# BichenWuUCB/squeezeDet

Hardware: NVIDIA H100
Metric: images/sec (1242x375, b=20) (higher is better)
Workload: dtype f32 (3xTF32 wgmma, fp32 accumulate)

## Files before the change

include/sqdet_b200.h:

```cpp
#ifndef SQDET_B200_H_
#define SQDET_B200_H_

#include <stdint.h>

#ifdef __cplusplus
extern "C" {
#endif

#define SQDET_OK                 0
#define SQDET_ERR_INVALID_ARG   (-1)
#define SQDET_ERR_CUDA          (-2)
#define SQDET_ERR_UNSUPPORTED   (-3)
#define SQDET_ERR_STATE         (-4)
#define SQDET_ERR_NOT_FOUND     (-5)
#define SQDET_ERR_OVERFLOW      (-6)

#define SQDET_PAD_SAME   0
#define SQDET_PAD_VALID  1

#define SQDET_MATH_FP32_SIMT   0
#define SQDET_MATH_TF32X3_TC   1

typedef struct sqdet_engine sqdet_engine;

// ... 32 lines not shown
                      int size, int stride, int relu, int conv_with_bias, int* out);
int sqdet_add_pool(sqdet_engine* e, const char* layer_name, int src, int size,
                   int stride, int padding, int* out);
int sqdet_add_fire(sqdet_engine* e, const char* layer_name, int src, int s1x1,
                   int e1x1, int e3x3, int* out);
int sqdet_add_add_relu(sqdet_engine* e, const char* name, int a, int b, int* out);
int sqdet_set_preds(sqdet_engine* e, int preds, const double* anchor_box, int64_t num_anchors);
int sqdet_finalize(sqdet_engine* e);

int sqdet_num_params(sqdet_engine* e);
int sqdet_param_info(sqdet_engine* e, int index, char* name_buf, int name_cap,
                     int64_t shape[4], int* ndim);
int sqdet_set_param(sqdet_engine* e, const char* name, const float* data,
                    const int64_t* shape, int ndim);

int sqdet_num_tensors(sqdet_engine* e);
int sqdet_tensor_info(sqdet_engine* e, int id, char* name_buf, int name_cap,
                      int64_t shape[4]);
int sqdet_read_tensor(sqdet_engine* e, int id, float* host_out);
int sqdet_num_ops(sqdet_engine* e);
int sqdet_op_info(sqdet_engine* e, int index, char* name_buf, int name_cap,
                  int64_t* flops, int64_t* params, int64_t* min_bytes);
int sqdet_op_k_split(sqdet_engine* e, int index);

int sqdet_forward(sqdet_engine* e, const float* images_dev, void* stream);
int sqdet_forward_n(sqdet_engine* e, const float* images_dev, int n, void* stream);
int sqdet_forward_u8(sqdet_engine* e, const uint8_t* images_dev, int n, void* stream);
int sqdet_forward_profiled(sqdet_engine* e, const float* images_dev, void* stream,
                           float* op_ms);
int sqdet_results_dev(sqdet_engine* e, float** det_boxes, float** det_probs,
                      int64_t** det_class, sqdet_det** dets, int32_t** counts,
                      int32_t* max_dets);
int sqdet_detect(sqdet_engine* e, const float* images, float* det_boxes,
                 float* det_probs, int64_t* det_class, sqdet_det* dets,
                 int32_t* counts, void* stream);
#define SQDET_IMG_F32 0
#define SQDET_IMG_U8  1
int sqdet_set_bgr_means(sqdet_engine* e, const double bgr_means[3]);
int sqdet_submit(sqdet_engine* e, const void* images, int img_type, sqdet_det* dets,
                 int32_t* counts);
int sqdet_wait(sqdet_engine* e);
int sqdet_submit_frames(sqdet_engine* e, const uint8_t* const* frames,
                        const int32_t* heights, const int32_t* widths, int order,
                        int rescale, sqdet_det* dets, int32_t* counts);
int sqdet_submit_frames_n(sqdet_engine* e, int n, const uint8_t* const* frames,
                          const int32_t* heights, const int32_t* widths, int order,
// ... 28 lines not shown
int sqdet_comm_unique_id(void* id128);
int sqdet_comm_init(sqdet_engine* e, int nranks, int rank, const void* id128);
int sqdet_comm_attach(sqdet_engine* e, void* nccl_comm, int nranks, int rank);
int sqdet_comm_destroy(sqdet_engine* e);
int sqdet_set_gather_in_forward(sqdet_engine* e, int on);
int sqdet_allgather(sqdet_engine* e, void* nccl_comm, void* stream);
int sqdet_gathered_dev(sqdet_engine* e, void** gathered_dev, int64_t* bytes_per_rank,
                       int32_t* nranks);

int sqdet_conv2d(const float* x_dev, const float* w_hwio_dev, const float* bias_dev,
                 const float* scale_dev, const float* shift_dev, float* y_dev,
                 int B, int H, int W, int Cin, int Cout, int size, int stride,
                 int padding, int relu, int y_cstride, int y_coff, int math_mode,
                 void* stream);
int sqdet_conv2d_k_split(const float* x_dev, const float* w_hwio_dev, const float* bias_dev,
                         const float* scale_dev, const float* shift_dev, float* y_dev,
                         int B, int H, int W, int Cin, int Cout, int size, int stride,
                         int padding, int relu, int y_cstride, int y_coff, int math_mode,
                         int k_split, void* stream);
int sqdet_fire(const float* x_dev, const float* w_sq_dev, const float* b_sq_dev,
               const float* w_e1_dev, const float* b_e1_dev, const float* w_e3_dev,
               const float* b_e3_dev, float* y_dev, int B, int H, int W, int Cin, int S,
               int E1, int E3, int math_mode, void* stream);
int sqdet_maxpool_nhwc(const float* x_dev, float* y_dev, int B, int H, int W, int C,
                       int size, int stride, int padding, void* stream);
#define SQDET_PRE_RESIZE_THEN_SUB 0
#define SQDET_PRE_SUB_THEN_RESIZE 1
int sqdet_preprocess_u8(const uint8_t* src_dev, int src_h, int src_w, float* dst_dev,
                        int dst_h, int dst_w, const double* bgr_means, int order,
                        void* stream);
int sqdet_interpret(const float* preds_dev, const float* anchors_f32_dev,
                    float* det_boxes_dev, float* det_probs_dev, int64_t* det_class_dev,
                    int B, int grid_h, int grid_w, int anchors_per_grid, int classes,
                    int image_width, int image_height, float exp_thresh, void* stream);
int sqdet_topk_nms(const float* boxes_dev, const float* probs_dev,
                   const int64_t* cls_dev, int B, int A, int classes, int top_n,
                   float prob_thresh, float nms_thresh, sqdet_det* dets_dev,
                   int32_t* counts_dev, int max_dets, void* stream);
int sqdet_merge_tiles(const float* boxes_dev, const float* probs_dev, const int64_t* cls_dev,
                      int A, int t, const int32_t* tile_frames, const int32_t* tile_xy, int n,
                      int classes, int top_n, float prob_thresh, float nms_thresh,
                      sqdet_det* dets_dev, int32_t* counts_dev, int max_dets, void* stream);
typedef struct sqdet_draw_style {
  int32_t            classes;
  const char* const* class_names;
  const uint8_t*     class_bgr;
// ... 60 lines not shown
```

squeezedet_b200/_lib.py:

```python
from __future__ import annotations

import ctypes as C
import os

import numpy as np

_HERE = os.path.dirname(os.path.abspath(__file__))
LIB_PATH = os.path.join(_HERE, 'lib', 'libsqdet_b200.so')

OK = 0
PAD_SAME, PAD_VALID = 0, 1
MATH_FP32_SIMT, MATH_TF32X3_TC = 0, 1
IMG_F32, IMG_U8 = 0, 1
_PAD = {'SAME': PAD_SAME, 'VALID': PAD_VALID}


class SqdetError(RuntimeError):
  def __init__(self, code, msg):
    super().__init__('sqdet error %d: %s' % (code, msg))
    self.code = code


class Det(C.Structure):
  _fields_ = [('anchor', C.c_int32), ('cls', C.c_int32), ('prob', C.c_float),
# ... 35 lines not shown

SIGNATURES = {
    'sqdet_last_error': (C.c_char_p, []),
    'sqdet_version': (C.c_char_p, []),
    'sqdet_device_count': (_i, []),
    'sqdet_create': (_i, [C.POINTER(Config), _i, C.POINTER(_vp)]),
    'sqdet_destroy': (_i, [_vp]),
    'sqdet_add_conv': (_i, [_vp, C.c_char_p, _i, _i, _i, _i, _i, _i, _ip]),
    'sqdet_add_conv_bn': (_i, [_vp, C.c_char_p, _i, _i, _i, _i, _i, _i, _ip]),
    'sqdet_add_pool': (_i, [_vp, C.c_char_p, _i, _i, _i, _i, _ip]),
    'sqdet_add_fire': (_i, [_vp, C.c_char_p, _i, _i, _i, _i, _ip]),
    'sqdet_add_add_relu': (_i, [_vp, C.c_char_p, _i, _i, _ip]),
    'sqdet_set_preds': (_i, [_vp, _i, _vp, _i64]),
    'sqdet_finalize': (_i, [_vp]),
    'sqdet_num_params': (_i, [_vp]),
    'sqdet_param_info': (_i, [_vp, _i, C.c_char_p, _i, _i64p, _ip]),
    'sqdet_set_param': (_i, [_vp, C.c_char_p, _fp, _i64p, _i]),
    'sqdet_num_tensors': (_i, [_vp]),
    'sqdet_tensor_info': (_i, [_vp, _i, C.c_char_p, _i, _i64p]),
    'sqdet_read_tensor': (_i, [_vp, _i, _fp]),
    'sqdet_num_ops': (_i, [_vp]),
    'sqdet_op_info': (_i, [_vp, _i, C.c_char_p, _i, _i64p, _i64p, _i64p]),
    'sqdet_op_k_split': (_i, [_vp, _i]),
    'sqdet_forward': (_i, [_vp, _fp, _vp]),
    'sqdet_forward_n': (_i, [_vp, _fp, _i, _vp]),
    'sqdet_forward_u8': (_i, [_vp, _vp, _i, _vp]),
    'sqdet_forward_profiled': (_i, [_vp, _fp, _vp, _fp]),
    'sqdet_results_dev': (_i, [_vp, C.POINTER(_vp), C.POINTER(_vp), C.POINTER(_vp),
                               C.POINTER(_vp), C.POINTER(_vp), C.POINTER(C.c_int32)]),
    'sqdet_detect': (_i, [_vp, _fp, _fp, _fp, _fp, _fp, _fp, _vp]),
    'sqdet_set_bgr_means': (_i, [_vp, _vp]),
    'sqdet_submit': (_i, [_vp, _vp, _i, _vp, _vp]),
    'sqdet_wait': (_i, [_vp]),
    'sqdet_submit_frames': (_i, [_vp, _vp, _vp, _vp, _i, _i, _vp, _vp]),
    'sqdet_submit_frames_n': (_i, [_vp, _i, _vp, _vp, _vp, _i, _i, _vp, _vp]),
    'sqdet_forward_frames_u8': (_i, [_vp, _i, _vp, _vp, _vp, _vp, _i, _i, _vp]),
    'sqdet_forward_frames_nv12': (_i, [_vp, _i, _vp, _vp, _vp, _vp, _vp, _vp, _vp, _i, _i, _vp]),
    'sqdet_forward_frames': (_i, [_vp, _i, _i, _vp, _vp, _vp, _vp, _vp, _i, _i, _vp]),
    'sqdet_forward_tiles': (_i, [_vp, _i, _i, _vp, _vp, _vp, _vp, _i, _vp, _i, _vp]),
    'sqdet_tile_results_dev': (_i, [_vp, C.POINTER(_vp), C.POINTER(_vp), C.POINTER(C.c_int32)]),
    'sqdet_set_box_scale': (_i, [_vp, _vp]),
    'sqdet_launches_per_forward': (_i, [_vp]),
    'sqdet_engine_stream': (_vp, [_vp]),
    'sqdet_comm_unique_id': (_i, [_vp]),
    'sqdet_comm_init': (_i, [_vp, _i, _i, _vp]),
    'sqdet_comm_attach': (_i, [_vp, _vp, _i, _i]),
    'sqdet_comm_destroy': (_i, [_vp]),
    'sqdet_set_gather_in_forward': (_i, [_vp, _i]),
    'sqdet_allgather': (_i, [_vp, _vp, _vp]),
    'sqdet_gathered_dev': (_i, [_vp, C.POINTER(_vp), C.POINTER(C.c_int64),
                                C.POINTER(C.c_int32)]),
    'sqdet_fire': (_i, [_fp] * 8 + [_i] * 8 + [_vp]),
    'sqdet_conv2d': (_i, [_fp, _fp, _fp, _fp, _fp, _fp] + [_i] * 12 + [_vp]),
    'sqdet_conv2d_k_split': (_i, [_fp, _fp, _fp, _fp, _fp, _fp] + [_i] * 13 + [_vp]),
    'sqdet_maxpool_nhwc': (_i, [_fp, _fp] + [_i] * 7 + [_vp]),
    'sqdet_preprocess_u8': (_i, [_vp, _i, _i, _fp, _i, _i, _vp, _i, _vp]),
    'sqdet_interpret': (_i, [_fp, _fp, _fp, _fp, _fp] + [_i] * 7 + [_f, _vp]),
    'sqdet_topk_nms': (_i, [_fp, _fp, _fp, _i, _i, _i, _i, _f, _f, _fp, _fp, _i, _vp]),
    'sqdet_merge_tiles': (_i, [_fp, _fp, _fp, _i, _i, _vp, _vp, _i, _i, _i, _f, _f, _fp, _fp, _i,
                               _vp]),
    'sqdet_draw_dets': (_i, [_i, _i, _vp, _vp, _vp, _vp, _vp, _vp, _vp, _i, C.POINTER(DrawStyle),
                             _vp]),
    'sqdet_jpeg_max_bytes': (_i64, [_i, _i]),
    'sqdet_jpeg_scratch_bytes': (_i64, [_i, _vp, _vp, _vp]),
    'sqdet_encode_jpeg': (_i, [_i, _i, _vp, _vp, _vp, _vp, _vp, _i, _vp, _i64, _vp, _vp, _i64, _vp]),
    'sqdet_jpeg_parse': (_i, [_vp, _i64, C.POINTER(JpegInfo)]),
    'sqdet_jpeg_decode_staging_bytes': (_i64, [_i, _vp, _vp]),
    'sqdet_jpeg_decode_scratch_bytes': (_i64, [_i, _vp, _vp]),
    'sqdet_decode_jpeg': (_i, [_i, _vp, _vp, _vp, _vp, _vp, _i64, _vp, _i64, _vp, _vp]),
    'sqdet_jpeg_decode_set_subsequence_bits': (_i, [_i]),
    'sqdet_malloc': (_i, [_i, _i64, C.POINTER(_vp)]),
    'sqdet_free': (_i, [_i, _vp]),
    'sqdet_malloc_host': (_i, [_i64, C.POINTER(_vp)]),
    'sqdet_free_host': (_i, [_vp]),
    'sqdet_memcpy_h2d': (_i, [_vp, _vp, _i64, _vp]),
    'sqdet_memcpy_d2h': (_i, [_vp, _vp, _i64, _vp]),
    'sqdet_stream_sync': (_i, [_i, _vp]),
# ... 141 lines not shown
```

squeezedet_b200/csrc/conv_tc.cu:

```cuda
#include <cuda.h>
#include <cuda_runtime.h>
#include <stdint.h>
#include <stdlib.h>
#include <string.h>

#include <vector>

#include "common.cuh"
#include "conv_tc.cuh"

namespace sqdet {
namespace {

constexpr int TILE_M = 128;
constexpr int NUM_THREADS = 256;
constexpr int STAGES = 3;
constexpr int MAX_CHUNKS = 32;
constexpr int FT_W = 16, FQ_W = FT_W + 2, FQ_P = 10 * FQ_W;

enum TcMode { TC_ROWS, TC_GATHER, TC_HALO, TC_FIRE };

struct TcChunk {
  int ksize, pad_t, pad_l;
  int nk;
  int ncount;
  int y_off;
  int p_off;
  long long w_off;
};

struct TcParams {
  CUtensorMap amap, amap1;
  const float* x;
  float* y;
  const float* w;
  const float* bias;
  const float* scale;
  const float* shift;
  int B, H, W, Cin, Ho, Wo, stride, relu, y_cstride;
  long long M;
  int tiles_w, tiles_h;
  int nchunks;
  TcChunk chunks[MAX_CHUNKS];
};

__device__ __forceinline__ uint32_t smem_u32(const void* p) {
  return static_cast<uint32_t>(__cvta_generic_to_shared(p));
}
__device__ __forceinline__ void cp_async4(uint32_t dst, const void* src, bool valid) {
  asm volatile("cp.async.ca.shared.global [%0], [%1], 4, %2;" ::"r"(dst), "l"(src),
// ... 275 lines not shown
  return {rest / tiles_h, rest % tiles_h * 8, tx * FT_W};
}

__device__ __forceinline__ float finish(const TcParams& p, const TcChunk& ch, int c, float v) {
  if (p.bias) v += p.bias[ch.p_off + c];
  if (p.scale) v = v * p.scale[ch.p_off + c] + p.shift[ch.p_off + c];
  if (p.relu) v = fmaxf(v, 0.f);
  return v;
}

template <typename Value>
__device__ __forceinline__ void store_pair(float* yrow, int c, int ncount, bool pair, Value value) {
  if (pair && c + 1 < ncount) {
    *reinterpret_cast<float2*>(yrow + c) = make_float2(value(c), value(c + 1));
  } else {
    if (c < ncount) yrow[c] = value(c);
    if (c + 1 < ncount) yrow[c + 1] = value(c + 1);
  }
}
__device__ __forceinline__ bool rows_pair_aligned(const TcParams& p, const TcChunk& ch) {
  return ((p.y_cstride | ch.y_off) & 1) == 0 && (reinterpret_cast<uintptr_t>(p.y) & 7) == 0;
}

template <int NT, int KC, int MODE, bool KSPLIT = false>
__global__ void __launch_bounds__(NUM_THREADS, 2)
conv_tc_kernel(const __grid_constant__ TcParams p) {
  static_assert(!KSPLIT || MODE == TC_HALO, "the K split walks halo-mode channel chunks");
  constexpr int NACC = NT / 2;
  constexpr int WST = 2 * NT * KC;
  constexpr uint32_t W_BYTES = WST * 4, TILE_BYTES = TILE_M * KC * 4, HALO_BYTES = FQ_P * KC * 4;
  constexpr int HROWS = halo_rows(KC);
  extern __shared__ __align__(16) uint8_t smem_raw[];
  float* const smem = reinterpret_cast<float*>(smem_raw + ((1024 - (smem_u32(smem_raw) & 1023)) & 1023));
  float* const sa = smem + STAGES * WST;
  uint64_t* const full = reinterpret_cast<uint64_t*>(sa + STAGES * TILE_M * KC);
  uint64_t* const empty = full + STAGES;

  const TcChunk& ch = p.chunks[blockIdx.y];
  const int tid = threadIdx.x;
  const int wg = tid >> 7, wq = (tid >> 5) & 3, lane = tid & 31, g = lane >> 2, t = lane & 3;
  const float* wch = p.w + ch.w_off;
  int k0 = 0, nk = ch.nk;
  const int taps = ch.ksize * ch.ksize;
  if (KSPLIT) {
    const int nc = ch.nk / taps, S = gridDim.z, z = blockIdx.z;
    k0 = z * nc / S * taps;
    nk = (z + 1) * nc / S * taps - k0;
    wch += (size_t)k0 * WST;
  }

// ... 64 lines not shown
  const int arow0 = wg * 64 + wq * 16 + g;
  const int r = wg * 4 + wq;
  float acc[2][NACC], sum[NACC];
#pragma unroll
  for (int i = 0; i < NACC; ++i) acc[0][i] = acc[1][i] = sum[i] = 0.f;

  for (int kk = 0; kk < nk; ++kk) {
    if (kk + STAGES - 1 < nk) load_stage(kk + STAGES - 1);
    const int s = ring_wait_full(full, kk);

    const float* tile = sa + s * TILE_M * KC;
    int prow = arow0;
    if (MODE == TC_HALO && taps > 1) {
      const int c = kk / 9, tap = kk - c * 9;
      tile = sa + (c & 1) * HROWS * KC;
      prow = (r + tap / 3) * FQ_W + g + tap % 3;
    }
    mma_chunk<NT, KC, NT != 72>(
        [&](int ks, uint32_t(&ahi)[4], uint32_t(&alo)[4]) { load_split_swz<KC>(tile, prow, ks, t, ahi, alo); },
        smem_u32(smem + s * WST), acc, sum);
    ring_release(empty, kk);
  }

  if constexpr (KSPLIT) {
    static_assert(TILE_M * NT <= STAGES * (WST + TILE_M * KC), "the partial tile fits in the ring");
    float* const part = smem;
    __syncthreads();
#pragma unroll
    for (int h = 0; h < 2; ++h)
#pragma unroll
      for (int j = 0; j < NT / 8; ++j)
        *reinterpret_cast<float2*>(part + (arow0 + 8 * h) * NT + 8 * j + 2 * t) =
            make_float2(sum[4 * j + 2 * h], sum[4 * j + 2 * h + 1]);
    cluster_sync();
    constexpr int G = TILE_M * NT / 4;
    const int S = gridDim.z, z = blockIdx.z;
    const HaloTile tl = halo_tile(p.tiles_w, p.tiles_h);
    for (int i = z * G / S + tid; i < (z + 1) * G / S; i += NUM_THREADS) {
      const uint32_t at = smem_u32(part + 4 * i);
      float4 v = ld_cluster_f4(at, 0);
      for (int q = 1; q < S; ++q) {
        const float4 u = ld_cluster_f4(at, q);
        v.x += u.x, v.y += u.y, v.z += u.z, v.w += u.w;
      }
      const int px = 4 * i / NT, c0 = 4 * i % NT;
      const int oy = tl.oy0 + px / FT_W, ox = tl.ox0 + px % FT_W;
      if (oy >= p.Ho || ox >= p.Wo) continue;
      float* yrow = p.y + (((size_t)tl.n * p.Ho + oy) * p.Wo + ox) * p.y_cstride + ch.y_off;
      const float vs[4] = {v.x, v.y, v.z, v.w};
#pragma unroll
      for (int e = 0; e < 4; ++e)
        if (c0 + e < ch.ncount) yrow[c0 + e] = finish(p, ch, c0 + e, vs[e]);
    }
    cluster_sync();
  } else {
    const bool pair = rows_pair_aligned(p, ch);
#pragma unroll
    for (int h = 0; h < 2; ++h) {
      long long m = m0 + arow0 + 8 * h;
      if (MODE == TC_HALO) {
        const HaloTile tl = halo_tile(p.tiles_w, p.tiles_h);
        const int oy = tl.oy0 + r, ox = tl.ox0 + g + 8 * h;
        if (oy >= p.Ho || ox >= p.Wo) continue;
        m = ((long long)tl.n * p.Ho + oy) * p.Wo + ox;
      } else if (m >= p.M) {
        continue;
      }
      float* yrow = p.y + (size_t)m * p.y_cstride + ch.y_off;
#pragma unroll
      for (int j = 0; j < NT / 8; ++j)
        store_pair(yrow, 8 * j + 2 * t, ch.ncount, pair,
                   [&](int c) { return finish(p, ch, c, sum[4 * j + 2 * h + (c & 1)]); });
    }
  }
}

constexpr int FS = 16;
constexpr int FQ_ROWS = 192;

__host__ __device__ constexpr int fire_stage_floats(int KCI) { return 2 * FS * KCI + FQ_ROWS * KCI; }
constexpr size_t fire_smem_bytes(int KCI) {
  return 1024 + ((size_t)STAGES * fire_stage_floats(KCI) + FQ_ROWS * (FS + 4)) * sizeof(float) +
         2 * STAGES * sizeof(uint64_t);
}

template <int KCI>
__global__ void __launch_bounds__(NUM_THREADS, 2)
fire_tc_kernel(const __grid_constant__ TcParams p) {
  constexpr int QP = FS + 4;
  constexpr int SQW = 2 * FS * KCI;
  constexpr int STAGE = fire_stage_floats(KCI);
  constexpr uint32_t SQW_BYTES = SQW * 4, HALO_BYTES = FQ_P * KCI * 4, EX_BYTES = 2 * 64 * FS * 4;
  static_assert(EX_BYTES <= (SQW + FQ_P * KCI) * 4, "expand tile fits before the zeroed rows");
  static_assert(SQW_BYTES % 1024 == 0 && STAGE * 4 % 1024 == 0, "A tiles keep the swizzle's alignment");
  extern __shared__ __align__(16) uint8_t smem_raw[];
// ... 138 lines not shown
}

TcKernel conv_tc_instance(int NT, int KC, int mode) {
  if (NT == 72) return mode == TC_HALO ? conv_tc_kernel<72, 32, TC_HALO> : conv_tc_kernel<72, 32, TC_ROWS>;
  if (mode == TC_GATHER) return conv_tc_instance<32, TC_GATHER>(NT);
  if (mode == TC_HALO)
    return KC == 32 ? conv_tc_instance<32, TC_HALO>(NT) : conv_tc_instance<16, TC_HALO>(NT);
  return KC == 32 ? conv_tc_instance<32, TC_ROWS>(NT) : conv_tc_instance<16, TC_ROWS>(NT);
}

struct PlanGroup {
  ConvGroup conv;
  int NT, KC, cin, chunk0;
};

}

struct TcImpl {
  TcParams prm{};
  int KC = 0;
  int mode = TC_ROWS;
  TcKernel kernel = nullptr;
  int ksplit = 1;
  size_t smem_bytes = 0;
  std::vector<PlanGroup> groups;
  int cout_total = 0;
  float* d_w = nullptr;
  float* d_bias = nullptr;
  float* d_scale = nullptr;
  float* d_shift = nullptr;
  long long w_floats = 0;
  const float* map_x = nullptr;
  int map_n = 0;
};

static inline float host_rn_tf32(float x) {
  uint32_t u;
  memcpy(&u, &x, 4);
  u = (u + 0x1000u) & 0xFFFFE000u;
  float r;
  memcpy(&r, &u, 4);
  return r;
}

static int pick_nt(const std::vector<ConvGroup>& groups, int KC, bool gather) {
  int best = 0;
// ... 83 lines not shown
  std::vector<int> poffs;
  int poff = 0;
  for (const auto& g : im->groups) poffs.push_back(poff), poff += g.conv.Cout;
  std::vector<size_t> order;
  for (int pass = 0; pass < 2; ++pass)
    for (size_t gi = 0; gi < im->groups.size(); ++gi)
      if ((im->mode == TC_HALO && im->groups[gi].conv.ksize == 3) == (pass == 0)) order.push_back(gi);
  int nch = 0;
  long long woff = 0;
  for (const size_t gi : order) {
    PlanGroup& g = im->groups[gi];
    g.chunk0 = nch;
    const int taps = g.conv.ksize * g.conv.ksize;
    const int nk = gather ? (taps * g.cin + g.KC - 1) / g.KC : taps * (g.cin / g.KC);
    for (int cb = 0; cb < g.conv.Cout; cb += g.NT, ++nch) {
      TcChunk& c = p.chunks[nch];
      c.ksize = g.conv.ksize;
      c.pad_t = gather ? pad_t : g.conv.ksize / 2;
      c.pad_l = gather ? pad_l : g.conv.ksize / 2;
      c.nk = nk;
      c.ncount = g.conv.Cout - cb < g.NT ? g.conv.Cout - cb : g.NT;
      c.y_off = g.conv.y_off + cb;
      c.p_off = poffs[gi] + cb;
      c.w_off = woff;
      woff += (long long)nk * 2 * g.NT * g.KC;
    }
  }
  p.nchunks = nch;
  im->cout_total = poff;
  im->w_floats = woff;
  cudaError_t ce = cudaFuncSetAttribute(im->kernel, cudaFuncAttributeMaxDynamicSharedMemorySize,
                                        (int)im->smem_bytes);
  if (ce != cudaSuccess) return cuda_fail(ce, "cudaFuncSetAttribute(tensor-core kernel)");
  SQ_CUDA(cudaMalloc(&im->d_w, sizeof(float) * (size_t)woff));
  SQ_CUDA(cudaMalloc(&im->d_bias, sizeof(float) * poff));
  SQ_CUDA(cudaMemset(im->d_bias, 0, sizeof(float) * poff));
  if (has_affine) {
    SQ_CUDA(cudaMalloc(&im->d_scale, sizeof(float) * poff));
    SQ_CUDA(cudaMalloc(&im->d_shift, sizeof(float) * poff));
  }
  p.w = im->d_w;
  p.bias = im->d_bias;
  p.scale = im->d_scale;
  p.shift = im->d_shift;
  return 1;
}
// ... 54 lines not shown
  int S = forced;
  if (!forced) {
    int dev = 0, sms = 0, per_sm = 0;
    SQ_CUDA(cudaGetDevice(&dev));
    SQ_CUDA(cudaDeviceGetAttribute(&sms, cudaDevAttrMultiProcessorCount, dev));
    SQ_CUDA(cudaOccupancyMaxActiveBlocksPerMultiprocessor(&per_sm, im->kernel, NUM_THREADS, im->smem_bytes));
    const long long ctas = grid_blocks(im, im->prm.B) * im->prm.nchunks;
    S = 1;
    long long best_waves = (ctas + per_sm * sms - 1) / (per_sm * sms);
    for (int s = 2; s <= MAX_KSPLIT && s * MIN_RANK_CHUNKS <= nc; ++s) {
      int clusters = 0;
      const ClusterLaunch l(dim3(1), im->smem_bytes, s, nullptr);
      SQ_CUDA(cudaOccupancyMaxActiveClusters(&clusters, split, &l.cfg));
      if (clusters < 1) continue;
      const long long waves = (ctas + clusters - 1) / clusters;
      if (waves * S < best_waves * s) S = s, best_waves = waves;
    }
  }
  if (S > 1) im->kernel = split;
  im->ksplit = S;
  return 1;
}

bool tc_conv_eligible(int Cin, int Cout, int size, int stride, int padding) {
  if (stride != 1 || padding != SQDET_PAD_SAME || (size != 1 && size != 3)) return false;
  return Cin % 16 == 0 && Cin >= 16 && Cout > 0;
}

int tc_conv_plan(TcConvPlan* plan, int B, int H, int W, int Cin, const std::vector<ConvGroup>& convs,
                 int stride, int padding, int relu, bool has_affine, int y_cstride, int k_split) {
  plan->impl = nullptr;
  const int size = convs[0].ksize;
  const bool gather = convs.size() == 1 && Cin == 3 && size == 3 && (stride == 1 || stride == 2) &&
                      convs[0].Cout > 0;
  if (!gather)
    for (const auto& g : convs)
      if (!tc_conv_eligible(Cin, g.Cout, g.ksize, stride, padding)) return 0;
  const Geom gh = tf_geometry(H, size, stride, padding);
  const Geom gw = tf_geometry(W, size, stride, padding);
  if (gh.out <= 0 || gw.out <= 0) return 0;
  const int KC = (gather || Cin % 32 == 0) ? 32 : 16;
  const int NT = pick_nt(convs, KC, gather);
  if (!NT) return 0;
  int mode = gather ? TC_GATHER : TC_ROWS;
  for (const auto& g : convs)
    if (!gather && g.ksize == 3) mode = TC_HALO;
  TcImpl* im = plan->impl = new TcImpl();
  im->KC = KC;
  im->mode = mode;
  im->kernel = conv_tc_instance(NT, KC, mode);
  im->smem_bytes = conv_smem_bytes(NT, KC);
  for (const auto& g : convs) im->groups.push_back({g, NT, KC, Cin, 0});
  int rc = plan_common(im, B, H, W, Cin, gh.out, gw.out, stride, gh.pad_before, gw.pad_before,
                       relu, has_affine, y_cstride);
  if (rc > 0 && NT == 72 && mode == TC_HALO) {
    rc = plan_ksplit(im, k_split);
  } else if (rc > 0 && k_split > 1) {
    rc = fail(SQDET_ERR_INVALID_ARG, "a K split needs a 72-wide 3x3 tensor-core plan");
  }
  if (rc <= 0) tc_conv_release(plan);
  return rc;
}

int tc_conv_k_split(const TcConvPlan& plan) { return plan.impl ? plan.impl->ksplit : 1; }

int tc_fire_plan(TcConvPlan* plan, int B, int H, int W, int Cin, int S, int E1, int E3) {
  plan->impl = nullptr;
  if (Cin % 16 || Cin < 16 || S != FS || E1 <= 0 || E3 <= 0) return 0;
  if ((E1 + 63) / 64 + (E3 + 63) / 64 > 16) return 0;
  const int KCI = Cin % 32 == 0 ? 32 : 16;
  TcImpl* im = plan->impl = new TcImpl();
  im->KC = KCI;
  im->mode = TC_FIRE;
  im->kernel = KCI == 32 ? fire_tc_kernel<32> : fire_tc_kernel<16>;
  im->smem_bytes = fire_smem_bytes(KCI);
  im->groups = {{{1, FS, 0}, FS, KCI, Cin, 0}, {{1, E1, 0}, 64, FS, FS, 0}, {{3, E3, E1}, 64, FS, FS, 0}};
  const int rc = plan_common(im, B, H, W, Cin, H, W, 1, 0, 0, 1, false, E1 + E3);
  if (rc <= 0) tc_conv_release(plan);
  return rc;
}

int tc_conv_pack_weights(TcConvPlan* plan, const std::vector<const float*>& w_hwio,
                         const std::vector<const float*>& bias) {
  TcImpl* im = plan->impl;
  std::vector<float> packed((size_t)im->w_floats, 0.f);
  for (size_t gi = 0; gi < im->groups.size(); ++gi) pack_group(im, im->groups[gi], w_hwio[gi], packed);
  SQ_CUDA(cudaMemcpy(im->d_w, packed.data(), packed.size() * sizeof(float), cudaMemcpyHostToDevice));
// ... 5 lines not shown
  }
  return SQDET_OK;
}

int tc_conv_set_affine(TcConvPlan* plan, const float* scale, const float* shift) {
  TcImpl* im = plan->impl;
  if (!im->d_scale) return fail(SQDET_ERR_STATE, "tc conv planned without an affine epilogue");
  SQ_CUDA(cudaMemcpy(im->d_scale, scale, sizeof(float) * im->cout_total, cudaMemcpyHostToDevice));
  SQ_CUDA(cudaMemcpy(im->d_shift, shift, sizeof(float) * im->cout_total, cudaMemcpyHostToDevice));
  return SQDET_OK;
}

int launch_conv_tc(const TcConvPlan& plan, const float* x_dev, float* y_dev, int n,
                   cudaStream_t stream) {
  TcImpl* im = plan.impl;
  if (n < 1 || n > im->prm.B) return fail(SQDET_ERR_INVALID_ARG, "launch_conv_tc: image count outside [1, B]");
  const int rc = update_maps(im, x_dev, n);
  if (rc) return rc;
  TcParams prm = im->prm;
  prm.x = x_dev;
  prm.y = y_dev;
  prm.B = n;
  prm.M = (long long)n * prm.Ho * prm.Wo;
  const dim3 grid((unsigned)grid_blocks(im, n), im->mode == TC_FIRE ? 1u : (unsigned)prm.nchunks);
  if (im->ksplit > 1) {
    const ClusterLaunch l(grid, im->smem_bytes, im->ksplit, stream);
    SQ_CUDA(cudaLaunchKernelEx(&l.cfg, im->kernel, prm));
  } else {
    im->kernel<<<grid, NUM_THREADS, im->smem_bytes, stream>>>(prm);
  }
  SQ_CHECK_LAUNCH(im->mode == TC_FIRE ? "fire_tc_kernel" : "conv_tc_kernel");
  return SQDET_OK;
}

void tc_conv_release(TcConvPlan* plan) {
  TcImpl* im = plan->impl;
  if (!im) return;
  cudaFree(im->d_w);
  cudaFree(im->d_bias);
  cudaFree(im->d_scale);
  cudaFree(im->d_shift);
  delete im;
  plan->impl = nullptr;
}

int tc_conv_oneshot(TcConvPlan* plan, const std::vector<const float*>& w_hwio_dev,
                    const std::vector<const float*>& bias_dev, const float* scale_dev,
// ... 32 lines not shown
```

squeezedet_b200/csrc/conv_tc.cuh:

```cuda
#pragma once
#include <cuda_runtime.h>
#include <stdint.h>

#include <vector>

namespace sqdet {

struct ConvGroup {
  int ksize, Cout, y_off;
};

struct TcImpl;

struct TcConvPlan {
  TcImpl* impl = nullptr;
};

bool tc_conv_eligible(int Cin, int Cout, int size, int stride, int padding);

int tc_conv_plan(TcConvPlan* plan, int B, int H, int W, int Cin, const std::vector<ConvGroup>& convs,
                 int stride, int padding, int relu, bool has_affine, int y_cstride, int k_split = 0);
int tc_conv_k_split(const TcConvPlan& plan);
int tc_fire_plan(TcConvPlan* plan, int B, int H, int W, int Cin, int S, int E1, int E3);
int tc_conv_pack_weights(TcConvPlan* plan, const std::vector<const float*>& w_hwio,
                         const std::vector<const float*>& bias);
int tc_conv_set_affine(TcConvPlan* plan, const float* scale, const float* shift);
int launch_conv_tc(const TcConvPlan& plan, const float* x_dev, float* y_dev, int n,
                   cudaStream_t stream);
void tc_conv_release(TcConvPlan* plan);

int tc_conv_oneshot(TcConvPlan* plan, const std::vector<const float*>& w_hwio_dev,
                    const std::vector<const float*>& bias_dev, const float* scale_dev,
                    const float* shift_dev, const float* x_dev, float* y_dev, cudaStream_t stream);

}
```

squeezedet_b200/csrc/engine.cu:

```cuda
#include <cuda_runtime.h>
#include <dlfcn.h>
#include <math.h>
#include <stdio.h>
#include <stdlib.h>
#include <string.h>

#include <functional>
#include <map>
#include <memory>
#include <string>
#include <vector>

#include "common.cuh"
#include "conv_tc.cuh"

namespace sqdet {

static thread_local std::string g_last_error;

void set_error(const std::string& msg) { g_last_error = msg; }

int fail(int code, const std::string& msg) {
  g_last_error = msg;
  return code;
// ... 981 lines not shown
      by = B * A * 4 + B * (int64_t)e->max_dets * (int64_t)sizeof(sqdet_det);
    }
  }
  if (name_buf && name_cap > 0) {
    strncpy(name_buf, name.c_str(), (size_t)name_cap - 1);
    name_buf[name_cap - 1] = 0;
  }
  if (flops) *flops = fl;
  if (params) *params = pa;
  if (min_bytes) *min_bytes = by;
  return SQDET_OK;
}

int sqdet_op_k_split(sqdet_engine* e, int index) {
  if (!e || index < 0 || index >= (int)e->ops.size() + 2)
    return fail(SQDET_ERR_INVALID_ARG, "sqdet_op_k_split: bad index");
  int s = 1;
  if (index < (int)e->ops.size())
    for (const auto& l : e->ops[index].launches)
      if (l.kind == L_CONV_TC) s = std::max(s, tc_conv_k_split(l.tc));
  return s;
}

int sqdet_forward(sqdet_engine* e, const float* images_dev, void* stream) {
  return sqdet_forward_n(e, images_dev, e ? e->cfg.batch_size : 0, stream);
}

int sqdet_forward_n(sqdet_engine* e, const float* images_dev, int n, void* stream) {
  return forward_impl(e, images_dev, false, n, e ? e->box_scale : nullptr, (cudaStream_t)stream);
}

int sqdet_forward_u8(sqdet_engine* e, const uint8_t* images_dev, int n, void* stream) {
  return forward_impl(e, images_dev, true, n, e ? e->box_scale : nullptr, (cudaStream_t)stream);
}

int sqdet_forward_profiled(sqdet_engine* e, const float* images_dev, void* stream_v,
                           float* op_ms) {
  if (!e || !op_ms) return fail(SQDET_ERR_INVALID_ARG, "sqdet_forward_profiled: null argument");
  if (!e->finalized) return fail(SQDET_ERR_STATE, "sqdet_forward_profiled before sqdet_finalize");
  if (!images_dev) return fail(SQDET_ERR_INVALID_ARG, "null images pointer");
  cudaStream_t stream = (cudaStream_t)stream_v;
  DeviceGuard guard(e->device);
  int rc = prepare_params(e);
  if (rc) return rc;
  const int n = (int)e->ops.size() + 2;
  while ((int)e->prof_events.size() < n + 1) {
// ... 507 lines not shown
    int rc = tc_fire_plan(&plan, B, H, W, Cin, S, E1, E3);
    if (rc >= 0)
      rc = tc_conv_oneshot(&plan, {w_sq_dev, w_e1_dev, w_e3_dev}, {b_sq_dev, b_e1_dev, b_e3_dev},
                           nullptr, nullptr, x_dev, y_dev, stream);
    if (rc != 1) return rc;
  }
  float* q = nullptr;
  SQ_CUDA(cudaMalloc(&q, sizeof(float) * (size_t)B * H * W * S));
  int rc = sqdet_conv2d(x_dev, w_sq_dev, b_sq_dev, nullptr, nullptr, q, B, H, W, Cin, S, 1, 1,
                        SQDET_PAD_SAME, 1, S, 0, math_mode, stream_v);
  if (!rc)
    rc = sqdet_conv2d(q, w_e1_dev, b_e1_dev, nullptr, nullptr, y_dev, B, H, W, S, E1, 1, 1,
                      SQDET_PAD_SAME, 1, E1 + E3, 0, math_mode, stream_v);
  if (!rc)
    rc = sqdet_conv2d(q, w_e3_dev, b_e3_dev, nullptr, nullptr, y_dev, B, H, W, S, E3, 3, 1,
                      SQDET_PAD_SAME, 1, E1 + E3, E1, math_mode, stream_v);
  cudaError_t ce = cudaStreamSynchronize(stream);
  cudaFree(q);
  if (rc) return rc;
  if (ce != cudaSuccess) return cuda_fail(ce, "sqdet_fire sync");
  return SQDET_OK;
}

int sqdet_maxpool_nhwc(const float* x_dev, float* y_dev, int B, int H, int W, int C, int size,
                       int stride, int padding, void* stream) {
  if (!x_dev || !y_dev) return fail(SQDET_ERR_INVALID_ARG, "sqdet_maxpool_nhwc: null pointer");
  if (padding != SQDET_PAD_SAME && padding != SQDET_PAD_VALID)
    return fail(SQDET_ERR_INVALID_ARG, "sqdet_maxpool_nhwc: padding must be SAME(0) or VALID(1)");
  return launch_maxpool(x_dev, y_dev, B, H, W, C, size, stride, padding, (cudaStream_t)stream);
}

int sqdet_preprocess_u8(const uint8_t* src_dev, int src_h, int src_w, float* dst_dev, int dst_h,
                        int dst_w, const double* bgr_means, int order, void* stream) {
  if (!src_dev || !dst_dev || !bgr_means)
    return fail(SQDET_ERR_INVALID_ARG, "sqdet_preprocess_u8: null pointer");
  if (order != SQDET_PRE_RESIZE_THEN_SUB && order != SQDET_PRE_SUB_THEN_RESIZE)
    return fail(SQDET_ERR_INVALID_ARG, "sqdet_preprocess_u8: order must be 0 (demo) or 1 (eval)");
  const FrameSource f = {{src_dev}, {3 * (int64_t)src_w}, 0, 0, src_h, src_w};
  return launch_resize_meansub_frames(SQDET_FMT_BGR, &f, 1, dst_dev, dst_h, dst_w, bgr_means,
                                      order == SQDET_PRE_SUB_THEN_RESIZE, nullptr,
                                      (cudaStream_t)stream);
}

int sqdet_interpret(const float* preds_dev, const float* anchors_f32_dev, float* det_boxes_dev,
                    float* det_probs_dev, int64_t* det_class_dev, int B, int grid_h, int grid_w,
                    int anchors_per_grid, int classes, int image_width, int image_height,
// ... 67 lines not shown
```

squeezedet_b200/nn_skeleton.py:

```python
from __future__ import annotations

import ctypes as C

import numpy as np

from . import _lib
from ._lib import SqdetError
from .frames import ORDERS, PIXEL_FORMATS, frame_count, order_code, pack_frames


class GraphTensor:

  def __init__(self, model, name, tid=None, shape=None, fetch=None):
    self.model = model
    self.name = name
    self.id = tid
    self.shape = shape
    self.fetch = fetch

  def get_shape(self):
    return self.shape

  def __repr__(self):
    return 'GraphTensor(%r, shape=%r)' % (self.name, self.shape)
# ... 466 lines not shown
                                                ms.ctypes.data))
    return list(zip(self.op_table(), ms.tolist()))

  def op_table(self):
    rows = []
    for i in range(self._lib.sqdet_num_ops(self._engine)):
      buf = C.create_string_buffer(256)
      fl, pa, by = C.c_int64(), C.c_int64(), C.c_int64()
      _lib.check(self._lib.sqdet_op_info(self._engine, i, buf, 256, C.byref(fl),
                                         C.byref(pa), C.byref(by)))
      rows.append((buf.value.decode(), fl.value, pa.value, by.value))
    return rows

  def op_k_splits(self):
    out = {}
    for i, (name, _, _, _) in enumerate(self.op_table()):
      s = self._lib.sqdet_op_k_split(self._engine, i)
      if s < 0:
        _lib.check(s)
      if s > 1:
        out[name] = s
    return out

  def results_device(self):
    ptrs = [C.c_void_p() for _ in range(5)]
    md = C.c_int32()
    _lib.check(self._lib.sqdet_results_dev(self._engine, *[C.byref(p) for p in ptrs],
                                           C.byref(md)))
    keys = ('det_boxes', 'det_probs', 'det_class', 'dets', 'counts')
    out = {k: p.value for k, p in zip(keys, ptrs)}
    out['max_dets'] = int(md.value)
    return out

  def launches_per_forward(self):
    return self._lib.sqdet_launches_per_forward(self._engine)

  def filter_prediction(self, boxes, probs, cls_idx):
    mc = self.mc
    boxes = np.ascontiguousarray(np.asarray(boxes, dtype=np.float32)).reshape(-1, 4)
    probs = np.ascontiguousarray(np.asarray(probs, dtype=np.float32)).reshape(-1)
    cls_idx = np.ascontiguousarray(np.asarray(cls_idx, dtype=np.int64)).reshape(-1)
    n = len(probs)
    if n == 0:
      return [], [], []
    topn = 0 < mc.TOP_N_DETECTION < n
    cap = int(mc.TOP_N_DETECTION) if topn else min(n, 1024)
# ... 13 lines not shown
```

Baseline: 4849.

## Fold 1x1 expand chunks into 3x3 halo CTAs of fire expand pairs

When a halo-mode plan covers a 3x3 and a 1x1 expand group and the grid would exceed one wave, each 3x3 channel chunk CTA is paired with a 1x1 chunk. After finishing its 3x3 work, the CTA reuses the already loaded halo tile to compute the partner chunk, so the grid shrinks by the number of folded chunks. The aim is to cut wave-quantization tail and repeated activation loads, at the cost of uneven per-CTA work and a new kernel variant. Fold selection runs automatically by default using an occupancy query.

```diff
diff --git a/include/sqdet_b200.h b/include/sqdet_b200.h
--- a/include/sqdet_b200.h
+++ b/include/sqdet_b200.h
@@ -78,6 +78,7 @@
 int sqdet_op_info(sqdet_engine* e, int index, char* name_buf, int name_cap,
                   int64_t* flops, int64_t* params, int64_t* min_bytes);
 int sqdet_op_k_split(sqdet_engine* e, int index);
+int sqdet_op_folded(sqdet_engine* e, int index);
 
 int sqdet_forward(sqdet_engine* e, const float* images_dev, void* stream);
 int sqdet_forward_n(sqdet_engine* e, const float* images_dev, int n, void* stream);
@@ -152,6 +153,10 @@
                const float* w_e1_dev, const float* b_e1_dev, const float* w_e3_dev,
                const float* b_e3_dev, float* y_dev, int B, int H, int W, int Cin, int S,
                int E1, int E3, int math_mode, void* stream);
+int sqdet_expand_pair(const float* x_dev, const float* w_e1_dev, const float* b_e1_dev,
+                      const float* w_e3_dev, const float* b_e3_dev, float* y_dev,
+                      int B, int H, int W, int Cin, int E1, int E3, int y_cstride, int y_coff,
+                      int fold, int* folded, void* stream);
 int sqdet_maxpool_nhwc(const float* x_dev, float* y_dev, int B, int H, int W, int C,
                        int size, int stride, int padding, void* stream);
 #define SQDET_PRE_RESIZE_THEN_SUB 0
diff --git a/squeezedet_b200/_lib.py b/squeezedet_b200/_lib.py
--- a/squeezedet_b200/_lib.py
+++ b/squeezedet_b200/_lib.py
@@ -81,6 +81,7 @@
     'sqdet_num_ops': (_i, [_vp]),
     'sqdet_op_info': (_i, [_vp, _i, C.c_char_p, _i, _i64p, _i64p, _i64p]),
     'sqdet_op_k_split': (_i, [_vp, _i]),
+    'sqdet_op_folded': (_i, [_vp, _i]),
     'sqdet_forward': (_i, [_vp, _fp, _vp]),
     'sqdet_forward_n': (_i, [_vp, _fp, _i, _vp]),
     'sqdet_forward_u8': (_i, [_vp, _vp, _i, _vp]),
@@ -112,6 +113,7 @@
     'sqdet_fire': (_i, [_fp] * 8 + [_i] * 8 + [_vp]),
     'sqdet_conv2d': (_i, [_fp, _fp, _fp, _fp, _fp, _fp] + [_i] * 12 + [_vp]),
     'sqdet_conv2d_k_split': (_i, [_fp, _fp, _fp, _fp, _fp, _fp] + [_i] * 13 + [_vp]),
+    'sqdet_expand_pair': (_i, [_fp] * 6 + [_i] * 9 + [_ip, _vp]),
     'sqdet_maxpool_nhwc': (_i, [_fp, _fp] + [_i] * 7 + [_vp]),
     'sqdet_preprocess_u8': (_i, [_vp, _i, _i, _fp, _i, _i, _vp, _i, _vp]),
     'sqdet_interpret': (_i, [_fp, _fp, _fp, _fp, _fp] + [_i] * 7 + [_f, _vp]),
diff --git a/squeezedet_b200/csrc/conv_tc.cu b/squeezedet_b200/csrc/conv_tc.cu
--- a/squeezedet_b200/csrc/conv_tc.cu
+++ b/squeezedet_b200/csrc/conv_tc.cu
@@ -26,6 +26,7 @@
   int ncount;
   int y_off;
   int p_off;
+  int partner;
   long long w_off;
 };
 
@@ -347,10 +348,11 @@
   return ((p.y_cstride | ch.y_off) & 1) == 0 && (reinterpret_cast<uintptr_t>(p.y) & 7) == 0;
 }
 
-template <int NT, int KC, int MODE, bool KSPLIT = false>
+template <int NT, int KC, int MODE, bool KSPLIT = false, bool PARTNER = false>
 __global__ void __launch_bounds__(NUM_THREADS, 2)
 conv_tc_kernel(const __grid_constant__ TcParams p) {
   static_assert(!KSPLIT || MODE == TC_HALO, "the K split walks halo-mode channel chunks");
+  static_assert(!PARTNER || (MODE == TC_HALO && !KSPLIT && NT <= 64), "partners are halo-mode chunks");
   constexpr int NACC = NT / 2;
   constexpr int WST = 2 * NT * KC;
   constexpr uint32_t W_BYTES = WST * 4, TILE_BYTES = TILE_M * KC * 4, HALO_BYTES = FQ_P * KC * 4;
@@ -461,6 +463,44 @@
     ring_release(empty, kk);
   }
 
+  if (PARTNER && ch.partner >= 0) {
+    const int j0 = nk, j1 = nk + p.chunks[ch.partner].nk;
+    auto load_partner = [&](int j) {
+      const int s = ring_acquire(empty, j);
+      mbar_expect_tx(&full[s], W_BYTES);
+      bulk_load(smem_u32(smem + s * WST), wch + (size_t)j * WST, W_BYTES, &full[s]);
+    };
+    if (tid == 0) {
+#pragma unroll 1
+      for (int j = j0; j < j0 + STAGES - 1 && j < j1; ++j) load_partner(j);
+    }
+    const bool pair = rows_pair_aligned(p, ch);
+    const HaloTile tl = halo_tile(p.tiles_w, p.tiles_h);
+#pragma unroll
+    for (int h = 0; h < 2; ++h) {
+      const int oy = tl.oy0 + r, ox = tl.ox0 + g + 8 * h;
+      if (oy >= p.Ho || ox >= p.Wo) continue;
+      float* yrow = p.y + (((size_t)tl.n * p.Ho + oy) * p.Wo + ox) * p.y_cstride + ch.y_off;
+#pragma unroll
+      for (int j = 0; j < NT / 8; ++j)
+        store_pair(yrow, 8 * j + 2 * t, ch.ncount, pair,
+                   [&](int c) { return finish(p, ch, c, sum[4 * j + 2 * h + (c & 1)]); });
+    }
+#pragma unroll
+    for (int i = 0; i < NACC; ++i) acc[0][i] = acc[1][i] = sum[i] = 0.f;
+    for (int kk = j0; kk < j1; ++kk) {
+      if (tid == 0 && kk + STAGES - 1 < j1) load_partner(kk + STAGES - 1);
+      const int s = ring_wait_full(full, kk);
+      const float* tile = sa + ((kk - j0) & 1) * HROWS * KC;
+      int prow = (r + 1) * FQ_W + g + 1;
+      asm volatile("" : "+r"(prow));
+      mma_chunk<NT, KC>(
+          [&](int ks, uint32_t(&ahi)[4], uint32_t(&alo)[4]) { load_split_swz<KC>(tile, prow, ks, t, ahi, alo); },
+          smem_u32(smem + s * WST), acc, sum);
+      ring_release(empty, kk);
+    }
+  }
+
   if constexpr (KSPLIT) {
     static_assert(TILE_M * NT <= STAGES * (WST + TILE_M * KC), "the partial tile fits in the ring");
     float* const part = smem;
@@ -493,7 +533,8 @@
     }
     cluster_sync();
   } else {
-    const bool pair = rows_pair_aligned(p, ch);
+    const TcChunk& c = PARTNER && ch.partner >= 0 ? p.chunks[ch.partner] : ch;
+    const bool pair = rows_pair_aligned(p, c);
 #pragma unroll
     for (int h = 0; h < 2; ++h) {
       long long m = m0 + arow0 + 8 * h;
@@ -505,11 +546,11 @@
       } else if (m >= p.M) {
         continue;
       }
-      float* yrow = p.y + (size_t)m * p.y_cstride + ch.y_off;
+      float* yrow = p.y + (size_t)m * p.y_cstride + c.y_off;
 #pragma unroll
       for (int j = 0; j < NT / 8; ++j)
-        store_pair(yrow, 8 * j + 2 * t, ch.ncount, pair,
-                   [&](int c) { return finish(p, ch, c, sum[4 * j + 2 * h + (c & 1)]); });
+        store_pair(yrow, 8 * j + 2 * t, c.ncount, pair,
+                   [&](int col) { return finish(p, c, col, sum[4 * j + 2 * h + (col & 1)]); });
     }
   }
 }
@@ -694,6 +735,7 @@
   int mode = TC_ROWS;
   TcKernel kernel = nullptr;
   int ksplit = 1;
+  int folded = 0;
   size_t smem_bytes = 0;
   std::vector<PlanGroup> groups;
   int cout_total = 0;
@@ -823,6 +865,7 @@
       c.ncount = g.conv.Cout - cb < g.NT ? g.conv.Cout - cb : g.NT;
       c.y_off = g.conv.y_off + cb;
       c.p_off = poffs[gi] + cb;
+      c.partner = -1;
       c.w_off = woff;
       woff += (long long)nk * 2 * g.NT * g.KC;
     }
@@ -923,13 +966,56 @@
   return 1;
 }
 
+static int plan_fold(TcImpl* im, int forced) {
+  TcParams& p = im->prm;
+  if (im->mode != TC_HALO || im->groups.size() != 2 || im->groups[0].NT == 72) return 1;
+  const PlanGroup& g3 = im->groups[0].conv.ksize == 3 ? im->groups[0] : im->groups[1];
+  const PlanGroup& g1 = im->groups[0].conv.ksize == 3 ? im->groups[1] : im->groups[0];
+  if (g1.conv.ksize != 1 || p.chunks[g3.chunk0].nk > 2 * 9) return 1;
+  const int n3 = (g3.conv.Cout + g3.NT - 1) / g3.NT, n1 = (g1.conv.Cout + g1.NT - 1) / g1.NT;
+  const int pairs = n3 < n1 ? n3 : n1;
+  int f = forced < pairs ? forced : pairs;
+  if (forced < 0) {
+    int dev = 0, sms = 0, per_sm = 0;
+    SQ_CUDA(cudaGetDevice(&dev));
+    SQ_CUDA(cudaDeviceGetAttribute(&sms, cudaDevAttrMultiProcessorCount, dev));
+    SQ_CUDA(cudaOccupancyMaxActiveBlocksPerMultiprocessor(&per_sm, im->kernel, NUM_THREADS, im->smem_bytes));
+    const bool waves = grid_blocks(im, p.B) * p.nchunks > (long long)per_sm * sms;
+    f = waves && p.chunks[g3.chunk0].nk == 9 ? pairs : 0;
+  }
+  const long long kfloats = 2LL * g3.NT * g3.KC;
+  long long woff = 0;
+  for (int c = 0; c < p.nchunks - f; ++c) {
+    p.chunks[c].w_off = woff;
+    woff += p.chunks[c].nk * kfloats;
+    if (c < f) {
+      TcChunk& pc = p.chunks[p.nchunks - f + c];
+      p.chunks[c].partner = p.nchunks - f + c;
+      pc.w_off = woff;
+      woff += pc.nk * kfloats;
+    }
+  }
+  im->folded = f;
+  if (f) {
+    im->kernel = g3.NT == 64 ? (g3.KC == 32 ? conv_tc_kernel<64, 32, TC_HALO, false, true>
+                                            : conv_tc_kernel<64, 16, TC_HALO, false, true>)
+                 : g3.NT == 32 ? (g3.KC == 32 ? conv_tc_kernel<32, 32, TC_HALO, false, true>
+                                              : conv_tc_kernel<32, 16, TC_HALO, false, true>)
+                               : (g3.KC == 32 ? conv_tc_kernel<16, 32, TC_HALO, false, true>
+                                              : conv_tc_kernel<16, 16, TC_HALO, false, true>);
+    SQ_CUDA(cudaFuncSetAttribute(im->kernel, cudaFuncAttributeMaxDynamicSharedMemorySize, (int)im->smem_bytes));
+  }
+  return 1;
+}
+
 bool tc_conv_eligible(int Cin, int Cout, int size, int stride, int padding) {
   if (stride != 1 || padding != SQDET_PAD_SAME || (size != 1 && size != 3)) return false;
   return Cin % 16 == 0 && Cin >= 16 && Cout > 0;
 }
 
 int tc_conv_plan(TcConvPlan* plan, int B, int H, int W, int Cin, const std::vector<ConvGroup>& convs,
-                 int stride, int padding, int relu, bool has_affine, int y_cstride, int k_split) {
+                 int stride, int padding, int relu, bool has_affine, int y_cstride, int k_split,
+                 int fold) {
   plan->impl = nullptr;
   const int size = convs[0].ksize;
   const bool gather = convs.size() == 1 && Cin == 3 && size == 3 && (stride == 1 || stride == 2) &&
@@ -958,12 +1044,16 @@
     rc = plan_ksplit(im, k_split);
   } else if (rc > 0 && k_split > 1) {
     rc = fail(SQDET_ERR_INVALID_ARG, "a K split needs a 72-wide 3x3 tensor-core plan");
+  } else if (rc > 0) {
+    rc = plan_fold(im, fold);
   }
   if (rc <= 0) tc_conv_release(plan);
   return rc;
 }
 
 int tc_conv_k_split(const TcConvPlan& plan) { return plan.impl ? plan.impl->ksplit : 1; }
+
+int tc_conv_folded(const TcConvPlan& plan) { return plan.impl ? plan.impl->folded : 0; }
 
 int tc_fire_plan(TcConvPlan* plan, int B, int H, int W, int Cin, int S, int E1, int E3) {
   plan->impl = nullptr;
@@ -1015,7 +1105,7 @@
   prm.y = y_dev;
   prm.B = n;
   prm.M = (long long)n * prm.Ho * prm.Wo;
-  const dim3 grid((unsigned)grid_blocks(im, n), im->mode == TC_FIRE ? 1u : (unsigned)prm.nchunks);
+  const dim3 grid((unsigned)grid_blocks(im, n), im->mode == TC_FIRE ? 1u : (unsigned)(prm.nchunks - im->folded));
   if (im->ksplit > 1) {
     const ClusterLaunch l(grid, im->smem_bytes, im->ksplit, stream);
     SQ_CUDA(cudaLaunchKernelEx(&l.cfg, im->kernel, prm));
diff --git a/squeezedet_b200/csrc/conv_tc.cuh b/squeezedet_b200/csrc/conv_tc.cuh
--- a/squeezedet_b200/csrc/conv_tc.cuh
+++ b/squeezedet_b200/csrc/conv_tc.cuh
@@ -19,8 +19,10 @@
 bool tc_conv_eligible(int Cin, int Cout, int size, int stride, int padding);
 
 int tc_conv_plan(TcConvPlan* plan, int B, int H, int W, int Cin, const std::vector<ConvGroup>& convs,
-                 int stride, int padding, int relu, bool has_affine, int y_cstride, int k_split = 0);
+                 int stride, int padding, int relu, bool has_affine, int y_cstride, int k_split = 0,
+                 int fold = -1);
 int tc_conv_k_split(const TcConvPlan& plan);
+int tc_conv_folded(const TcConvPlan& plan);
 int tc_fire_plan(TcConvPlan* plan, int B, int H, int W, int Cin, int S, int E1, int E3);
 int tc_conv_pack_weights(TcConvPlan* plan, const std::vector<const float*>& w_hwio,
                          const std::vector<const float*>& bias);
diff --git a/squeezedet_b200/csrc/engine.cu b/squeezedet_b200/csrc/engine.cu
--- a/squeezedet_b200/csrc/engine.cu
+++ b/squeezedet_b200/csrc/engine.cu
@@ -1027,6 +1027,16 @@
   return s;
 }
 
+int sqdet_op_folded(sqdet_engine* e, int index) {
+  if (!e || index < 0 || index >= (int)e->ops.size() + 2)
+    return fail(SQDET_ERR_INVALID_ARG, "sqdet_op_folded: bad index");
+  int f = 0;
+  if (index < (int)e->ops.size())
+    for (const auto& l : e->ops[index].launches)
+      if (l.kind == L_CONV_TC) f += tc_conv_folded(l.tc);
+  return f;
+}
+
 int sqdet_forward(sqdet_engine* e, const float* images_dev, void* stream) {
   return sqdet_forward_n(e, images_dev, e ? e->cfg.batch_size : 0, stream);
 }
@@ -1580,6 +1590,24 @@
   return SQDET_OK;
 }
 
+int sqdet_expand_pair(const float* x_dev, const float* w_e1_dev, const float* b_e1_dev,
+                      const float* w_e3_dev, const float* b_e3_dev, float* y_dev, int B, int H, int W,
+                      int Cin, int E1, int E3, int y_cstride, int y_coff, int fold, int* folded,
+                      void* stream) {
+  if (!x_dev || !w_e1_dev || !w_e3_dev || !y_dev) return fail(SQDET_ERR_INVALID_ARG, "sqdet_expand_pair: null pointer");
+  if (B <= 0 || H <= 0 || W <= 0 || E1 <= 0 || E3 <= 0)
+    return fail(SQDET_ERR_INVALID_ARG, "sqdet_expand_pair: non-positive dimension");
+  if (int rc = check_conv_epilogue("sqdet_expand_pair", nullptr, nullptr, E1 + E3, y_cstride, y_coff)) return rc;
+  TcConvPlan plan;
+  int rc = tc_conv_plan(&plan, B, H, W, Cin, {{1, E1, y_coff}, {3, E3, y_coff + E1}}, 1, SQDET_PAD_SAME, 1,
+                        false, y_cstride, 0, fold);
+  if (rc == 0) return fail(SQDET_ERR_INVALID_ARG, "sqdet_expand_pair: Cin must be a positive multiple of 16");
+  if (rc < 0) return rc;
+  if (folded) *folded = tc_conv_folded(plan);
+  return tc_conv_oneshot(&plan, {w_e1_dev, w_e3_dev}, {b_e1_dev, b_e3_dev}, nullptr, nullptr, x_dev, y_dev,
+                         (cudaStream_t)stream);
+}
+
 int sqdet_maxpool_nhwc(const float* x_dev, float* y_dev, int B, int H, int W, int C, int size,
                        int stride, int padding, void* stream) {
   if (!x_dev || !y_dev) return fail(SQDET_ERR_INVALID_ARG, "sqdet_maxpool_nhwc: null pointer");
diff --git a/squeezedet_b200/nn_skeleton.py b/squeezedet_b200/nn_skeleton.py
--- a/squeezedet_b200/nn_skeleton.py
+++ b/squeezedet_b200/nn_skeleton.py
@@ -512,6 +512,16 @@
         out[name] = s
     return out
 
+  def op_folded(self):
+    out = {}
+    for i, (name, _, _, _) in enumerate(self.op_table()):
+      f = self._lib.sqdet_op_folded(self._engine, i)
+      if f < 0:
+        _lib.check(f)
+      if f > 0:
+        out[name] = f
+    return out
+
   def results_device(self):
     ptrs = [C.c_void_p() for _ in range(5)]
     md = C.c_int32()
```

After: 4871 (median of 6 runs). No clear change (+0.5%).
